# DerrickXuNu/CoBEVT

Hardware: AMD Instinct MI355X
Metric: bev_frames_per_sec (higher is better)
Workload: dtype bf16

## Files before the change

cobevt_amd/csrc/conv3x3.hip:

```cpp
#include <type_traits>

#include "common.hpp"
#include "f32_matrix.hpp"

namespace cobevt {

struct Conv3Params {
    const void* in;
    const void* wgt;
    const float* bias;
    const void* residual;
    void* out;
    int N, H, W, Cin;
    int Ho, Wo, Cout;
    int upsample;
    int act;
    int store_mode;
    int tiles_y, tiles_x, tiles_n;
    const void* in2 = nullptr;
    const float* bias2 = nullptr;
    int H2 = 0, W2 = 0, Cin2 = 0;
};

template <typename T, int NT, int NPX, int BN> struct Conv3Store {
    static constexpr int CH = Elem<T>::kChunk;
    static constexpr int CPP = BN / CH;
    static constexpr int ITEMS = NPX * CPP;
    static constexpr int NIT = (ITEMS + NT - 1) / NT;
    long off[NIT];
    uint4 rres[NIT];

    template <typename Coord>
    __device__ __forceinline__ void prepare(const Conv3Params& p, int tid, int n0, Coord coord) {
        const bool vec = (p.Cout % CH) == 0;
#pragma unroll
        for (int i = 0; i < NIT; ++i) {
            const int item = tid + i * NT;
            const int px = item / CPP, cj = item - px * CPP;
            const int col = n0 + cj * CH;
            int img = 0, oy = 0, ox = 0;
            rres[i] = make_uint4(0, 0, 0, 0);
            const bool ok = coord(px < NPX ? px : 0, img, oy, ox) & (item < ITEMS) & (col < p.Cout);
            const long o = (((long)img * p.Ho + oy) * p.Wo + ox) * p.Cout + col;
            off[i] = ok ? o : -1;
        }
        if (p.residual && vec) {
#pragma unroll
            for (int i = 0; i < NIT; ++i) rres[i] = *(const uint4*)((const T*)p.residual + (off[i] < 0 ? 0 : off[i]));
        }
    }

    __device__ __forceinline__ void finish(const Conv3Params& p, const float* stage, int srow, int tid, int n0) {
        T* out = (T*)p.out;
        const bool vec = (p.Cout % CH) == 0;
        float sv[NIT][CH];
#pragma unroll
        for (int i = 0; i < NIT; ++i) {
            const int item = tid + i * NT;
            const int px = item / CPP, cj = item - px * CPP;
            const float* src = stage + (px < NPX ? px : 0) * srow + cj * CH;
#pragma unroll
            for (int e = 0; e < CH; ++e) sv[i][e] = src[e];
        }
#pragma unroll
        for (int i = 0; i < NIT; ++i) {
            if (off[i] < 0) continue;
            const int item = tid + i * NT;
            const int px = item / CPP, cj = item - px * CPP;
            float v[8], rv[8];
#pragma unroll
            for (int e = 0; e < CH; ++e) v[e] = sv[i][e];
            if (vec) {
                if (p.residual) {
                    chunk_to_f32<T>(rres[i], rv);
#pragma unroll
                    for (int e = 0; e < CH; ++e) v[e] += rv[e];
                }
#pragma unroll
                for (int e = 0; e < CH; ++e) v[e] = p.act == 1 ? fmaxf(v[e], 0.f) : (p.act == 2 ? gelu_t<T>(v[e]) : v[e]);
                *(uint4*)(out + off[i]) = f32_to_chunk<T>(v);
            } else {
                const int col = n0 + cj * CH;
                for (int e = 0; e < CH && col + e < p.Cout; ++e) {
                    float x = v[e];
                    if (p.residual) x += load_elem<T>((const T*)p.residual, off[i] + e);
                    x = p.act == 1 ? fmaxf(x, 0.f) : (p.act == 2 ? gelu_t<T>(x) : x);
                    store_elem<T>(out, off[i] + e, x);
                }
            }
        }
    }
};

template <typename T, int NT, int NPX, int BN, typename Coord>
__device__ __forceinline__ void conv3_store_nhwc(const Conv3Params& p, const float* stage, int srow, int tid, int n0, Coord coord) {
    Conv3Store<T, NT, NPX, BN> st;
    st.prepare(p, tid, n0, coord);
    st.finish(p, stage, srow, tid, n0);
}

template <typename T, int BN, int KG> struct Conv3Cfg {
    static constexpr int TW = 16;
    static constexpr int TH = BN == 64 ? 16 : 8;
    static constexpr int PH = TH + 2, PW = TW + 2;
    static constexpr int PSTR = KG * 32 + 16;
    static constexpr int PROW = (PW * PSTR + 255) / 256 * 256;
    static constexpr int WSTR = KG * 32 + 16;
    static constexpr int PATCH_BYTES = PH * PROW;
    static constexpr int W_BYTES = BN * WSTR;
    static constexpr int SSTR = BN * 4 + 16;
    static constexpr int STAGE_BYTES = TH * TW * SSTR;
    static constexpr int MAIN_BYTES = PATCH_BYTES + 2 * W_BYTES;
    static constexpr int LDS_BYTES = MAIN_BYTES > STAGE_BYTES ? MAIN_BYTES : STAGE_BYTES;
};

constexpr int kConv3Threads = 512;

template <typename T, int BN, int KG>
__global__ __launch_bounds__(kConv3Threads) void conv3x3_kernel(Conv3Params p) {
    using C = Conv3Cfg<T, BN, KG>;
    constexpr int NT = kConv3Threads;
    constexpr int CH = Elem<T>::kChunk;
    constexpr int CC = KG * 32 / Elem<T>::kBytes;
    constexpr int TW = C::TW, TH = C::TH, PH = C::PH, PW = C::PW;
    constexpr int PSTR = C::PSTR, PROW = C::PROW, WSTR = C::WSTR;
    constexpr int PIECES = 2 * KG;
    constexpr int PATCH_ITEMS = PH * PW * PIECES;
    constexpr int P_IT = (PATCH_ITEMS + NT - 1) / NT;
    constexpr int W_ITEMS = BN * PIECES;
    constexpr int W_IT = (W_ITEMS + NT - 1) / NT;
    constexpr int WAVES_N = BN / 64;

    extern __shared__ __attribute__((aligned(16))) unsigned char smem[];
    unsigned char* patch = smem;
    unsigned char* wbuf = smem + C::PATCH_BYTES;

    int logical;
    {
        const int nblk = gridDim.x, bid = blockIdx.x, xcd = bid & 7, slot = bid >> 3;
        const int q = nblk >> 3, r = nblk & 7;
        logical = (xcd < r ? xcd * (q + 1) : r * (q + 1) + (xcd - r) * q) + slot;
    }
    const int tn = logical % p.tiles_n;
    int rest = logical / p.tiles_n;
    const int tx = rest % p.tiles_x; rest /= p.tiles_x;
    const int ty = rest % p.tiles_y;
    const int img = rest / p.tiles_y;
    const int oy0 = ty * TH, ox0 = tx * TW, n0 = tn * BN;

    const int tid = threadIdx.x, lane = tid & 63, wave = tid >> 6;
    const int h = lane >> 5, ql = lane & 31;
    const int wm = wave / WAVES_N, wn = wave % WAVES_N;
    const int nchunk = p.Cin / CC;
    const T* in = (const T*)p.in;
    const T* wg = (const T*)p.wgt;
    float ebias[2];
#pragma unroll
    for (int b = 0; b < 2; ++b) {
        const int c = n0 + wn * 64 + b * 32 + ql;
        ebias[b] = p.bias ? p.bias[p.bias && c < p.Cout ? c : 0] : 0.f;
        if (c >= p.Cout) ebias[b] = 0.f;
    }

    long pgoff[P_IT];
    int plds[P_IT];
    bool pzero[P_IT];
#pragma unroll
    for (int it = 0; it < P_IT; ++it) {
        const int item = tid + it * NT;
        pgoff[it] = 0;
        plds[it] = -1;
        pzero[it] = true;
        if (item < PATCH_ITEMS) {
            const int pix = item / PIECES, j = item - pix * PIECES;
            const int py = pix / PW, px = pix - py * PW;
            plds[it] = py * PROW + px * PSTR + j * 16;
            const int vy = oy0 - 1 + py, vx = ox0 - 1 + px;
            if (vy >= 0 && vy < p.Ho && vx >= 0 && vx < p.Wo) {
                const int sy = p.upsample ? (vy >> 1) : vy, sx = p.upsample ? (vx >> 1) : vx;
                pgoff[it] = (((long)img * p.H + sy) * p.W + sx) * p.Cin + j * CH;
                pzero[it] = false;
            }
        }
    }
    const T* wptr[W_IT];
    int wlds[W_IT];
    bool wzero[W_IT];
#pragma unroll
    for (int it = 0; it < W_IT; ++it) {
        const int item = (tid + it * NT) % W_ITEMS;
        const int row = item / PIECES, j = item - row * PIECES;
        const bool mine = tid + it * NT < W_ITEMS;
        wlds[it] = mine ? row * WSTR + j * 16 : -1;
        wzero[it] = n0 + row >= p.Cout;
        const int crow = n0 + row < p.Cout ? n0 + row : p.Cout - 1;
        wptr[it] = wg + ((size_t)crow * nchunk * 9 * CC + j * CH);
    }

    uint4 preg[P_IT];
    uint4 wregA[W_IT], wregB[W_IT];

    auto load_patch = [&](int chunk) {
#pragma unroll
        for (int it = 0; it < P_IT; ++it) preg[it] = *(const uint4*)(in + pgoff[it] + chunk * CC);
    };
    auto store_patch = [&]() {
#pragma unroll
        for (int it = 0; it < P_IT; ++it)
            if (plds[it] >= 0) *(uint4*)(patch + plds[it]) = pzero[it] ? make_uint4(0, 0, 0, 0) : stage_x_piece<T>(preg[it]);
    };
    auto load_w = [&](uint4 (&wreg)[W_IT], int step) {
#pragma unroll
        for (int it = 0; it < W_IT; ++it) wreg[it] = *(const uint4*)(wptr[it] + step * CC);
    };
    auto store_w = [&](const uint4 (&wreg)[W_IT], int buf) {
        unsigned char* wb = wbuf + buf * C::W_BYTES;
#pragma unroll
        for (int it = 0; it < W_IT; ++it)
            if (wlds[it] >= 0) *(uint4*)(wb + wlds[it]) = wzero[it] ? make_uint4(0, 0, 0, 0) : stage_w_piece<T>(wreg[it]);
    };

    f32x16 acc[2];
#pragma unroll
    for (int b = 0; b < 2; ++b)
#pragma unroll
        for (int r = 0; r < 16; ++r) acc[b][r] = 0.f;

    const int abase = (2 * wm + (ql >> 4)) * PROW + (ql & 15) * PSTR + h * 16;
    const int bbase = (wn * 64 + ql) * WSTR + h * 16;
    const int nsteps = nchunk * 9;

    auto body = [&](int step, int chunk, int tap, uint4 (&RI)[W_IT], uint4 (&RS)[W_IT], int buf) {
        const bool next_chunk = chunk + 1 < nchunk;
        load_w(RI, step + 2 < nsteps ? step + 2 : nsteps - 1);
        if (tap == 6 && next_chunk) load_patch(chunk + 1);
        const int kh = tap / 3, kw = tap - kh * 3;
        const unsigned char* pa = patch + kh * PROW + kw * PSTR + abase;
        const unsigned char* pb = wbuf + buf * C::W_BYTES + bbase;
#pragma unroll
        for (int g = 0; g < KG; ++g) {
            const uint4 af = *(const uint4*)(pa + g * 32);
            uint4 bf[2];
#pragma unroll
            for (int b = 0; b < 2; ++b) bf[b] = *(const uint4*)(pb + b * 32 * WSTR + g * 32);
#pragma unroll
            for (int b = 0; b < 2; ++b) mfma_kgroup_ss<T>(af, bf[b], acc[b]);
        }
        if (step + 1 < nsteps) store_w(RS, buf ^ 1);
        if (tap == 8 && next_chunk) {
            __syncthreads();
            store_patch();
        }
        __syncthreads();
    };

    load_patch(0);
    load_w(wregA, 0);
    store_patch();
    store_w(wregA, 0);
    load_w(wregB, nsteps > 1 ? 1 : 0);
    __syncthreads();
    {
        int chunk = 0, tap = 0;
        for (int step = 0; step < nsteps; step += 2) {
            body(step, chunk, tap, wregA, wregB, 0);
            if (++tap == 9) { tap = 0; ++chunk; }
            if (step + 1 < nsteps) {
                body(step + 1, chunk, tap, wregB, wregA, 1);
                if (++tap == 9) { tap = 0; ++chunk; }
            }
        }
    }

    float* stage = (float*)smem;
    constexpr int SROW = C::SSTR / 4;
#pragma unroll
    for (int b = 0; b < 2; ++b) {
        const int cl = wn * 64 + b * 32 + ql;
        const float bias = ebias[b];
#pragma unroll
        for (int r = 0; r < 16; ++r) {
            const int row = acc_row(r, lane);
            const int px = (2 * wm + (row >> 4)) * TW + (row & 15);
            stage[px * SROW + cl] = acc[b][r] + bias;
        }
    }
    __syncthreads();
    T* out = (T*)p.out;
    if (p.store_mode == 0) {
        conv3_store_nhwc<T, kConv3Threads, TH * TW, BN>(p, stage, SROW, tid, n0, [&](int px, int& im, int& oy, int& ox) {
            im = img; oy = oy0 + px / TW; ox = ox0 + (px % TW);
            return oy < p.Ho && ox < p.Wo;
        });
    } else {
        constexpr int QP = (TH / 2) * (TW / 2);
        const int ocn = BN * 4;
        const int cpp = ocn / CH;
        for (int item = tid; item < QP * cpp; item += kConv3Threads) {
            const int qp = item / cpp, cj = item - qp * cpp;
            const int qy = qp / (TW / 2), qx = qp % (TW / 2);
            const int oy2 = (oy0 >> 1) + qy, ox2 = (ox0 >> 1) + qx;
            if (oy2 >= (p.Ho >> 1) || ox2 >= (p.Wo >> 1)) continue;
            float v[8];
            bool any = false;
#pragma unroll
            for (int e = 0; e < CH; ++e) {
                const int oc = cj * CH + e, c = oc >> 2, q = oc & 3;
                const int px = (2 * qy + (q >> 1)) * TW + 2 * qx + (q & 1);
                float x = stage[px * SROW + c];
                x = p.act == 1 ? fmaxf(x, 0.f) : (p.act == 2 ? gelu_t<T>(x) : x);
                v[e] = x;
                any |= (n0 + c) < p.Cout;
            }
            if (!any) continue;
            const size_t o = (((size_t)img * (p.Ho >> 1) + oy2) * (p.Wo >> 1) + ox2) * (size_t)(p.Cout * 4) + (size_t)n0 * 4 + cj * CH;
            if (n0 + ((cj * CH + CH - 1) >> 2) < p.Cout && ((p.Cout * 4) % CH) == 0) *(uint4*)(out + o) = f32_to_chunk<T>(v);
            else for (int e = 0; e < CH; ++e) if (n0 + ((cj * CH + e) >> 2) < p.Cout) store_elem<T>(out, o + e, v[e]);
        }
    }
}

template <typename T, int BN, int KG>
static int launch_conv3(Conv3Params p, hipStream_t stream) {
    using C = Conv3Cfg<T, BN, KG>;
    p.tiles_y = (p.Ho + C::TH - 1) / C::TH;
    p.tiles_x = (p.Wo + 15) / 16;
    p.tiles_n = (p.Cout + BN - 1) / BN;
    const long blocks = (long)p.N * p.tiles_y * p.tiles_x * p.tiles_n;
    if (blocks <= 0 || blocks > 0x7fffffffL) return COBEVT_ERR_SHAPE;
    constexpr size_t lds = C::LDS_BYTES;
    cobevt::allow_dynamic_lds<conv3x3_kernel<T, BN, KG>>((int)lds);
    hipLaunchKernelGGL((conv3x3_kernel<T, BN, KG>), dim3((unsigned)blocks), dim3(kConv3Threads), lds, stream, p);
    return cobevt::launch_status();
}


#ifndef COBEVT_CONV3_PLOAD_TAP
#define COBEVT_CONV3_PLOAD_TAP 3
#endif
#ifndef COBEVT_CONV3_PSTORE_SPREAD
#define COBEVT_CONV3_PSTORE_SPREAD 1
#endif
#ifndef COBEVT_CONV3_PSTORE_FIRST
#define COBEVT_CONV3_PSTORE_FIRST 6
#endif
#ifndef COBEVT_CONV3_CONT
#define COBEVT_CONV3_CONT 1
#endif
#ifndef COBEVT_CONV3_CONT_LEAD
#define COBEVT_CONV3_CONT_LEAD 3
#endif
#ifndef COBEVT_CONV3_KNOCK
#define COBEVT_CONV3_KNOCK 0
#endif
#ifdef COBEVT_CONV3_TRACE
__device__ unsigned long long cobevt_conv3_trace[64];
__device__ unsigned long long cobevt_conv3_rt[3 * 2048];
#define COBEVT_TRACE_MARK(i) do { if (logical == 0 && tid == 0) cobevt_conv3_trace[(i)] = __builtin_readcyclecounter(); } while (0)
#define COBEVT_TRACE_RT(i) do { if (threadIdx.x == 0 && blockIdx.x < 2048) cobevt_conv3_rt[blockIdx.x * 3 + (i)] = (i) == 2 ? (unsigned long long)(__builtin_amdgcn_s_getreg((20 << 0) | (0 << 6) | (3 << 11)) & 15) : __builtin_amdgcn_s_memrealtime(); } while (0)
#else
#define COBEVT_TRACE_MARK(i) do {} while (0)
#define COBEVT_TRACE_RT(i) do {} while (0)
#endif

template <typename T, int MT, int WN, int KS, int S = 1, int NW = 8> struct Conv3SCfg {
    static constexpr int NT = 64 * NW, KG = 4, KGW = KG / KS;
    static constexpr bool HALF = NW == 4;
    static constexpr int BN = WN * 32;
    static constexpr int PW = S == 1 ? 18 : 33;
    static constexpr int SROWS = S == 1 ? 4 : 5;
    static constexpr int PSTR = KG * 32 + 16;
    static constexpr int PLANE = 17 * PSTR;
    static constexpr int PROW = ((S == 1 ? PW * PSTR : 2 * PLANE) + 255) / 256 * 256;
    static constexpr int STRIP_BYTES = SROWS * PROW;
    static constexpr int PATCH_BYTES = MT * STRIP_BYTES;
    static constexpr int SSTR = BN * 4 + 16;
    static constexpr int STAGE_BYTES = MT * 32 * SSTR;
    static constexpr int MAIN_BYTES = (S == 1 && !HALF ? 2 : 1) * PATCH_BYTES;
    static constexpr int LDS_BYTES = MAIN_BYTES > STAGE_BYTES ? MAIN_BYTES : STAGE_BYTES;
    static_assert(WN * KS == NW && (NW == 8 || (NW == 4 && S == 1)), "eight waves, or four (stride 1)");
};

template <typename T, int MT, int WN, int KS, int S, int NW, bool DS = false>
__global__ __launch_bounds__(64 * NW, NW == 4 ? 2 : 1) void conv3x3_strips_kernel(Conv3Params p) {
    static_assert(!DS || (Elem<T>::kIsBf16 && S == 1 && NW == 8), "the shortcut form is bf16 / stride 1 / eight waves");
    using C = Conv3SCfg<T, MT, WN, KS, S, NW>;
    constexpr bool HALF = C::HALF;
    constexpr int NT = C::NT, KG = C::KG, KGW = C::KGW, BN = C::BN, PW = C::PW;
    constexpr int CH = Elem<T>::kChunk;
    constexpr int CC = KG * 32 / Elem<T>::kBytes;
    constexpr int PSTR = C::PSTR, PROW = C::PROW, STRIP = C::STRIP_BYTES;
    constexpr int PIECES = 2 * KG;
    constexpr int STRIP_ITEMS = C::SROWS * PW * PIECES;
    constexpr int PATCH_ITEMS = MT * STRIP_ITEMS;
    constexpr int P_IT = S == 1 ? (PATCH_ITEMS + NT - 1) / NT : 1;
    constexpr int PF = 2, R = 3;
    constexpr bool PACK = kXPack<T, KGW>;
    constexpr bool PACK3 = kXPack3<T, KGW>;
    constexpr int KGA = (PACK || PACK3) ? KGW / 2 : KGW;
    constexpr int RA = PACK3 ? 2 : 3;
    constexpr bool CONT = COBEVT_CONV3_CONT && S == 1 && !HALF && Elem<T>::kIsBf16 && (KGA == 1 || KGA == 2) && MT <= 5;
    constexpr int TB = CONT ? (9 * KGA - 2) / KGA : 9;

    extern __shared__ __attribute__((aligned(16))) unsigned char smem[];
    unsigned char* patch = smem;
    COBEVT_TRACE_RT(0);
    COBEVT_TRACE_RT(2);

    int logical;
    {
        const int nblk = gridDim.x, bid = blockIdx.x, xcd = bid & 7, slot = bid >> 3;
        const int q = nblk >> 3, r = nblk & 7;
        logical = (xcd < r ? xcd * (q + 1) : r * (q + 1) + (xcd - r) * q) + slot;
    }
    const int tn = logical % p.tiles_n;
    const int q0 = (logical / p.tiles_n) * MT;
    const int n0 = tn * BN;
    const int per_img = p.tiles_y * p.tiles_x;
    const int nstrips = p.N * per_img;

    const int tid = threadIdx.x, lane = tid & 63, wave = tid >> 6;
    const int h = lane >> 5, ql = lane & 31;
    const int wn = wave % WN, ks = wave / WN;
    const int nchunk = p.Cin / CC;
    const int nchunk2 = DS ? p.Cin2 / CC : 0;
    const int nsteps = nchunk * 9 + nchunk2;
    const T* in = (const T*)p.in;

    __shared__ __attribute__((aligned(16))) int stab[8 * 4];
    __shared__ __attribute__((aligned(16))) float sbias[BN];
    __shared__ __attribute__((aligned(16))) float sbias2[DS ? BN : 4];
    if (tid >= NT - BN) {
        const int c = n0 + tid - (NT - BN);
        sbias[tid - (NT - BN)] = (p.bias && c < p.Cout) ? p.bias[c] : 0.f;
        if (DS) sbias2[tid - (NT - BN)] = (p.bias2 && c < p.Cout) ? p.bias2[c] : 0.f;
    }
    if (tid < MT) {
        const int q = q0 + tid;
        const bool ok = q < nstrips;
        const int img = ok ? q / per_img : 0, rem = ok ? q - img * per_img : 0;
        const int sy = rem / p.tiles_x, sx = rem - sy * p.tiles_x;
        *(int4*)&stab[tid * 4] = make_int4(img, sy, sx, ok ? 1 : 0);
    }
    __syncthreads();

    int pgoff[P_IT];
    int plds[P_IT];
#pragma unroll
    for (int it = 0; it < P_IT; ++it) {
        const int item = tid + it * NT;
        pgoff[it] = 0;
        plds[it] = -1;
        if (S == 1 && item < PATCH_ITEMS) {
            const int s = item / STRIP_ITEMS, r = item - s * STRIP_ITEMS;
            const int pix = r / PIECES, j = r - pix * PIECES;
            const int py = pix / PW, px = pix - py * PW;
            int lds = s * STRIP + py * PROW + px * PSTR + (PACK ? packed_piece_offset(j) : PACK3 ? packed3_piece_offset(j) : j * 16);
            const int4 sc = *(const int4*)&stab[s * 4];
            const int img = sc.x, sy = sc.y, sx = sc.z;
            const int vy = sy * 2 - 1 + py, vx = sx * 16 - 1 + px;
            const bool valid = (sc.w != 0) & (vy >= 0) & (vy < p.Ho) & (vx >= 0) & (vx < p.Wo);
            const int yy = p.upsample ? (vy >> 1) : vy, xx = p.upsample ? (vx >> 1) : vx;
            pgoff[it] = valid ? ((img * p.H + yy) * p.W + xx) * p.Cin + j * CH : 0;
            plds[it] = valid ? lds : (lds | (1 << 30));
        }
    }
    const uint4* wq = (const uint4*)p.wgt + ((size_t)(n0 / 32 + wn) * nsteps) * (KG * 64) + ks * KGW * 64 + lane;

    uint4 preg[P_IT];
    auto load_patch = [&](int chunk) {
#pragma unroll
        for (int it = 0; it < P_IT; ++it) preg[it] = *(const uint4*)(in + pgoff[it] + chunk * CC);
    };
    auto store_patch = [&](unsigned char* dst) {
#pragma unroll
        for (int it = 0; it < P_IT; ++it)
            if (plds[it] >= 0) {
                if constexpr (PACK) *(uint2*)(dst + (plds[it] & 0x3fffffff)) = (plds[it] >> 30) ? make_uint2(0, 0) : pack_f16_hi(preg[it]);
                else if constexpr (PACK3) store_piece_packed3(dst + (plds[it] & 0x3fffffff), preg[it], (plds[it] >> 30) != 0);
                else *(uint4*)(dst + (plds[it] & 0x3fffffff)) = (plds[it] >> 30) ? make_uint4(0, 0, 0, 0) : stage_x_piece<T>(preg[it]);
            }
    };
    constexpr int PSF = CONT ? TB - 3 : COBEVT_CONV3_PSTORE_FIRST;
    constexpr int PSN = TB - PSF;
    auto store_patch_part = [&](unsigned char* dst, int part) {
#pragma unroll
        for (int it = 0; it < P_IT; ++it)
            if (it % PSN == part && plds[it] >= 0) {
                if constexpr (PACK) *(uint2*)(dst + (plds[it] & 0x3fffffff)) = (plds[it] >> 30) ? make_uint2(0, 0) : pack_f16_hi(preg[it]);
                else if constexpr (PACK3) store_piece_packed3(dst + (plds[it] & 0x3fffffff), preg[it], (plds[it] >> 30) != 0);
                else *(uint4*)(dst + (plds[it] & 0x3fffffff)) = (plds[it] >> 30) ? make_uint4(0, 0, 0, 0) : stage_x_piece<T>(preg[it]);
            }
    };
    auto load_b = [&](uint4 (&b)[KGW], int step) {
#pragma unroll
        for (int g = 0; g < KGW; ++g) b[g] = wq[(size_t)step * (KG * 64) + g * 64];
    };
    auto fill_patch_s2 = [&](int chunk) {
        constexpr int BATCH = 8;
        for (int base = 0; base < PATCH_ITEMS; base += BATCH * NT) {
            uint4 v[BATCH];
            int dst[BATCH];
#pragma unroll
            for (int u = 0; u < BATCH; ++u) {
                const int item = base + u * NT + tid;
                dst[u] = -1;
                v[u] = make_uint4(0, 0, 0, 0);
                if (item < PATCH_ITEMS) {
                    const int st = item / STRIP_ITEMS, r = item - st * STRIP_ITEMS;
                    const int pix = r / PIECES, j = r - pix * PIECES;
                    const int py = pix / PW, px = pix - py * PW;
                    dst[u] = st * STRIP + py * PROW + (px & 1) * C::PLANE + (px >> 1) * PSTR + (PACK ? packed_piece_offset(j) : PACK3 ? packed3_piece_offset(j) : j * 16);
                    const int4 sc = *(const int4*)&stab[st * 4];
                    if (sc.w) {
                        const int img = sc.x, sy = sc.y, sx = sc.z;
                        const int vy = sy * 4 - 1 + py, vx = sx * 32 - 1 + px;
                        if (vy >= 0 && vy < p.H && vx >= 0 && vx < p.W)
                            v[u] = *(const uint4*)(in + ((img * p.H + vy) * p.W + vx) * p.Cin + j * CH + chunk * CC);
                    }
                }
            }
#pragma unroll
            for (int u = 0; u < BATCH; ++u)
                if (dst[u] >= 0) {
                    if constexpr (PACK) *(uint2*)(patch + dst[u]) = pack_f16_hi(v[u]);
                    else if constexpr (PACK3) store_piece_packed3(patch + dst[u], v[u], false);
                    else *(uint4*)(patch + dst[u]) = stage_x_piece<T>(v[u]);
                }
        }
    };

    f32x16 acc[MT];
#pragma unroll
    for (int a = 0; a < MT; ++a)
#pragma unroll
        for (int r = 0; r < 16; ++r) acc[a][r] = 0.f;

    const int abase = (ql >> 4) * S * PROW + (ql & 15) * PSTR + (PACK3 ? h * 32 + ks * KGA * 64 : h * 16 + ks * KGA * 32);

    uint4 bq[R][KGW];
    COBEVT_TRACE_MARK(0);
    if (S == 1) load_patch(0);
#pragma unroll
    for (int s = 0; s < PF; ++s) load_b(bq[s], s < nsteps ? s : nsteps - 1);
    float* stage = (float*)smem;
    constexpr int SROW = C::SSTR / 4;
    auto reduce_ksplit = [&](const float* bias_lds, bool trace) {
        const int c0 = wn * 32 + 4 * h;
        float4 bias4[4];
#pragma unroll
        for (int k = 0; k < 4; ++k) bias4[k] = *(const float4*)&bias_lds[c0 + 8 * k];
        if (trace) COBEVT_TRACE_MARK(57);
#pragma unroll
        for (int r = 0; r < KS; ++r) {
#pragma unroll
            for (int a = 0; a < MT; ++a) {
                if (((a + KS - r) % KS) != ks) continue;
#pragma unroll
                for (int k = 0; k < 4; ++k) {
                    float4* d = (float4*)(stage + (a * 32 + ql) * SROW + c0 + 8 * k);
                    float4 v = make_float4(acc[a][4 * k], acc[a][4 * k + 1], acc[a][4 * k + 2], acc[a][4 * k + 3]);
                    if (r == 0) {
                        v.x += bias4[k].x; v.y += bias4[k].y; v.z += bias4[k].z; v.w += bias4[k].w;
                    } else {
                        const float4 o = *d;
                        v.x += o.x; v.y += o.y; v.z += o.z; v.w += o.w;
                    }
                    *d = v;
                }
            }
            __syncthreads();
            if (trace && r == 0) COBEVT_TRACE_MARK(58);
        }
    };
    if (S == 1) store_patch(patch);
    else fill_patch_s2(0);
    __syncthreads();
    COBEVT_TRACE_MARK(1);
    constexpr bool EARLY_RES = S == 1 && Elem<T>::kIsBf16 && MT <= 5;
    Conv3Store<T, NT, MT * 32, BN> st;
    auto coord = [&](int px, int& im, int& oy, int& ox) {
        const int4 sc = *(const int4*)&stab[(px >> 5) * 4];
        im = sc.x;
        oy = sc.y * 2 + ((px >> 4) & 1); ox = sc.z * 16 + (px & 15);
        return (sc.w != 0) & (oy < p.Ho) & (ox < p.Wo);
    };
    constexpr int PLT = (S == 1 && !HALF) ? (CONT ? PSF - COBEVT_CONV3_CONT_LEAD : COBEVT_CONV3_PLOAD_TAP) : 0;
    uint4 af[RA][MT];
    uint4 al[PACK3 ? RA : 1][PACK3 ? MT : 1];
    auto read_a_from = [&](const unsigned char* pb, int slot, int n) {
        const int t2 = n / KGA, g2 = n - t2 * KGA;
        const int kh2 = t2 / 3, kw2 = t2 - kh2 * 3;
        const int toff = S == 1 ? kh2 * PROW + kw2 * PSTR : kh2 * PROW + (kw2 & 1) * C::PLANE + (kw2 >> 1) * PSTR;
        const unsigned char* pn = pb + toff + abase + g2 * (PACK3 ? 64 : 32);
#pragma unroll
        for (int a = 0; a < MT; ++a) {
            af[slot][a] = *(const uint4*)(pn + a * STRIP);
            if constexpr (PACK3) al[slot][a] = *(const uint4*)(pn + a * STRIP + 16);
        }
    };
    if (CONT) {
        read_a_from(patch, 0, 0);
        read_a_from(patch, 1, 1);
        __builtin_amdgcn_sched_barrier(0);
    }
    auto run_chunk = [&](int chunk, auto last_tag) {
        constexpr bool LAST = decltype(last_tag)::value;
        const bool more = chunk + 1 < nchunk;
        unsigned char* pbuf = patch + (S == 1 && !HALF ? (chunk & 1) * C::PATCH_BYTES : 0);
        unsigned char* pother = patch + (S == 1 && !HALF ? ((chunk & 1) ^ 1) * C::PATCH_BYTES : 0);
        if (S == 1 && PLT == 0 && !(COBEVT_CONV3_KNOCK & 8)) load_patch(more ? chunk + 1 : chunk);
        constexpr int NG = 9 * KGA;
        auto read_a = [&](int slot, int n) { read_a_from(pbuf, slot, n); };
        if (!CONT) {
            read_a(0, 0);
            if (RA == 3) read_a(1, 1);
            __builtin_amdgcn_sched_barrier(0);
        }
#pragma unroll
        for (int tap = 0; tap < 9; ++tap) {
            const int step = chunk * 9 + tap;
            if (chunk < 4) COBEVT_TRACE_MARK(2 + chunk * 9 + tap);
            if (CONT && tap == TB) {
                __syncthreads();
                __builtin_amdgcn_sched_barrier(0);
            }
#ifdef COBEVT_CONV3_SETPRIO
            if ((tap ^ ks) & 1) __builtin_amdgcn_s_setprio(3); else __builtin_amdgcn_s_setprio(0);
#endif
            if (!(COBEVT_CONV3_KNOCK & 1) || chunk == 0)
                load_b(bq[(tap + PF) % R], step + PF < nsteps ? step + PF : nsteps - 1);
            if (S == 1 && PLT > 0 && tap == PLT) {
                if (LAST) { if (EARLY_RES && p.store_mode == 0) st.prepare(p, tid, n0, coord); }
                else if (!(COBEVT_CONV3_KNOCK & 8)) load_patch(more ? chunk + 1 : chunk);
            }
            __builtin_amdgcn_sched_barrier(0);
#pragma unroll
            for (int g = 0; g < KGA; ++g) {
                const int n = tap * KGA + g;
                if (n + RA - 1 < NG) { if (!(COBEVT_CONV3_KNOCK & 4) || chunk == 0) read_a((n + RA - 1) % RA, n + RA - 1); }
                else if (CONT && !LAST && !(COBEVT_CONV3_KNOCK & 4)) read_a_from(pother, (n + RA - 1) % RA, n + RA - 1 - NG);
                uint4 wpk = make_uint4(0, 0, 0, 0), wlo = make_uint4(0, 0, 0, 0);
                if constexpr (PACK) wpk = pack_f16_pair(bq[tap % R][(2 * g) % KGW], bq[tap % R][(2 * g + 1) % KGW]);
                if constexpr (PACK3) split_w_pair(bq[tap % R][(2 * g) % KGW], bq[tap % R][(2 * g + 1) % KGW], wpk, wlo);
#pragma unroll
                for (int a = 0; a < MT; ++a) {
                    if (COBEVT_CONV3_KNOCK & 2) acc[a][0] += __uint_as_float((af[n % RA][a].x ^ bq[tap % R][g].x) & 0x3fffffffu);
                    else if constexpr (PACK) mfma_f16_packed(wpk, af[n % RA][a], acc[a]);
                    else if constexpr (PACK3) mfma_3term(wpk, wlo, af[n % RA][a], al[PACK3 ? n % RA : 0][PACK3 ? a : 0], acc[a]);
                    else mfma_kgroup_xs<T>(bq[tap % R][g], af[n % RA][a], acc[a]);
                }
                if (Elem<T>::kIsBf16 && (n + 2 < NG || (CONT && !LAST))) {
#pragma unroll
                    for (int a = 0; a < MT; ++a) {
                        __builtin_amdgcn_sched_group_barrier(0x100, 1, 0);
                        __builtin_amdgcn_sched_group_barrier(0x008, 1, 0);
                    }
                }
                __builtin_amdgcn_sched_barrier(0);
            }
            if (S == 1 && !HALF && more && !LAST && !(COBEVT_CONV3_KNOCK & 8)) {
                if (COBEVT_CONV3_PSTORE_SPREAD || CONT) {
                    if (tap >= PSF && tap < TB) { store_patch_part(pother, tap - PSF); __builtin_amdgcn_sched_barrier(0); }
                } else if (tap == 6) {
                    store_patch(pother);
                    __builtin_amdgcn_sched_barrier(0);
                }
            }
        }
        if (chunk < 4) COBEVT_TRACE_MARK(41 + 2 * chunk);
#ifdef COBEVT_CONV3_TRACE
        if (logical == 0 && lane == 0 && chunk == 0) {
            cobevt_conv3_trace[49 + wave] = __builtin_readcyclecounter();
            cobevt_conv3_trace[57 + wave > 63 ? 63 : 57 + wave] = 0;
            unsigned hw = __builtin_amdgcn_s_getreg((4 << 0) | (0 << 6) | (31 << 11));
            cobevt_conv3_trace[49 + wave] |= (unsigned long long)((hw >> 4) & 3) << 60;
        }
#endif
        if (!CONT) __syncthreads();
        if (HALF && more) {
            store_patch(pbuf);
            __syncthreads();
        }
        if (chunk < 4) COBEVT_TRACE_MARK(42 + 2 * chunk);
    };
    constexpr int XI = MT * 32 * PIECES, X_IT = DS ? (XI + NT - 1) / NT : 1, XCH = MT * 32 * PSTR;
    int xoff[X_IT], xlds[X_IT];
    const T* in2 = (const T*)p.in2;
    uint4 xr[2][X_IT];
    auto load_x = [&](uint4 (&x)[X_IT], int e) {
#pragma unroll
        for (int it = 0; it < X_IT; ++it) x[it] = *(const uint4*)(in2 + xoff[it] + e * CC);
    };
    auto store_x = [&](const uint4 (&x)[X_IT], int e) {
#pragma unroll
        for (int it = 0; it < X_IT; ++it)
            if (xlds[it] >= 0) *(uint4*)(patch + e * XCH + (xlds[it] & 0x3fffffff)) = (xlds[it] >> 30) ? make_uint4(0, 0, 0, 0) : x[it];
    };
    if (S == 1) {
        for (int chunk = 0; chunk + 1 < nchunk; ++chunk) run_chunk(chunk, std::false_type{});
        if constexpr (DS) {
#pragma unroll
            for (int it = 0; it < X_IT; ++it) {
                const int item = tid + it * NT;
                xoff[it] = 0;
                xlds[it] = -1;
                if (item < XI) {
                    const int pi = item / PIECES, j = item - pi * PIECES;
                    const int4 sc = *(const int4*)&stab[(pi >> 5) * 4];
                    const int oy = sc.y * 2 + ((pi >> 4) & 1), ox = sc.z * 16 + (pi & 15);
                    const bool valid = (sc.w != 0) & (oy < p.Ho) & (ox < p.Wo);
                    xoff[it] = valid ? ((sc.x * p.H2 + 2 * oy) * p.W2 + 2 * ox) * p.Cin2 + j * CH : 0;
                    xlds[it] = (pi * PSTR + j * 16) | (valid ? 0 : (1 << 30));
                }
            }
            load_x(xr[0], 0);
            load_x(xr[1], nchunk2 > 1 ? 1 : 0);
        }
        if (PLT == 0 && EARLY_RES && p.store_mode == 0) st.prepare(p, tid, n0, coord);
        __builtin_amdgcn_sched_barrier(0);
        run_chunk(nchunk - 1, std::true_type{});
    } else {
#pragma unroll 1
        for (int chunk = 0; chunk < nchunk; ++chunk) {
            if (chunk > 0) {
                fill_patch_s2(chunk);
                __syncthreads();
            }
            run_chunk(chunk, std::false_type{});
        }
    }
    if constexpr (DS) {
        for (int e0 = 0; e0 < nchunk2; e0 += 2) {
            if (e0 > 0) {
                load_x(xr[0], e0);
                load_x(xr[1], e0 + 1 < nchunk2 ? e0 + 1 : e0);
            }
            store_x(xr[0], e0);
            if (e0 + 1 < nchunk2) store_x(xr[1], e0 + 1);
        }
        __syncthreads();
        {
            const int c0 = wn * 32 + 4 * h;
            float4 bias4[4];
#pragma unroll
            for (int k = 0; k < 4; ++k) bias4[k] = *(const float4*)&sbias2[c0 + 8 * k];
            const uint4* wd = (const uint4*)p.wgt + ((size_t)(n0 / 32 + wn) * nsteps + nchunk * 9) * (KG * 64) + lane;
            uint4 bw[4][KG];
#pragma unroll
            for (int e = 0; e < 4; ++e)
                if (e < nchunk2) {
#pragma unroll
                    for (int g = 0; g < KG; ++g) bw[e][g] = wd[(size_t)e * (KG * 64) + g * 64];
                }
#pragma unroll
            for (int a = 0; a < MT; ++a) {
                if ((a % KS) != ks) continue;
                f32x16 dacc;
#pragma unroll
                for (int r = 0; r < 16; ++r) dacc[r] = 0.f;
                const unsigned char* xa = patch + (a * 32 + ql) * PSTR + h * 16;
#pragma unroll
                for (int e = 0; e < 4; ++e) {
                    if (e >= nchunk2) continue;
                    uint4 ax[KG];
#pragma unroll
                    for (int g = 0; g < KG; ++g) ax[g] = *(const uint4*)(xa + e * XCH + g * 32);
#pragma unroll
                    for (int g = 0; g < KG; ++g) mfma_kgroup_xs<T>(bw[e][g], ax[g], dacc);
                }
#pragma unroll
                for (int k = 0; k < 4; ++k) {
                    const uint32_t lo = pack_bf2(dacc[4 * k] + bias4[k].x, dacc[4 * k + 1] + bias4[k].y);
                    const uint32_t hi = pack_bf2(dacc[4 * k + 2] + bias4[k].z, dacc[4 * k + 3] + bias4[k].w);
                    acc[a][4 * k] += __uint_as_float(lo << 16);
                    acc[a][4 * k + 1] += __uint_as_float(lo & 0xffff0000u);
                    acc[a][4 * k + 2] += __uint_as_float(hi << 16);
                    acc[a][4 * k + 3] += __uint_as_float(hi & 0xffff0000u);
                }
            }
        }
        __syncthreads();
    }
    COBEVT_TRACE_MARK(38);

    reduce_ksplit(sbias, true);
    COBEVT_TRACE_MARK(39);
    T* out = (T*)p.out;
    if (p.store_mode == 0) {
        if (!EARLY_RES) st.prepare(p, tid, n0, coord);
        st.finish(p, stage, SROW, tid, n0);
    } else {
        const int cpp = BN * 4 / CH;
        for (int item = tid; item < MT * 8 * cpp; item += NT) {
            const int qp = item / cpp, cj = item - qp * cpp;
            const int s = qp >> 3, qx = qp & 7;
            const int4 sc = *(const int4*)&stab[s * 4];
            if (!sc.w) continue;
            const int img = sc.x, sy = sc.y, sx = sc.z;
            const int oy2 = sy, ox2 = sx * 8 + qx;
            if (oy2 >= (p.Ho >> 1) || ox2 >= (p.Wo >> 1)) continue;
            float v[8];
            bool any = false;
#pragma unroll
            for (int e = 0; e < CH; ++e) {
                const int oc = cj * CH + e, c = oc >> 2, qd = oc & 3;
                const int px = s * 32 + (qd >> 1) * 16 + 2 * qx + (qd & 1);
                float x = stage[px * SROW + c];
                x = p.act == 1 ? fmaxf(x, 0.f) : (p.act == 2 ? gelu_t<T>(x) : x);
                v[e] = x;
                any |= (n0 + c) < p.Cout;
            }
            if (!any) continue;
            const size_t o = (((size_t)img * (p.Ho >> 1) + oy2) * (p.Wo >> 1) + ox2) * (size_t)(p.Cout * 4) + (size_t)n0 * 4 + cj * CH;
            if (n0 + ((cj * CH + CH - 1) >> 2) < p.Cout && ((p.Cout * 4) % CH) == 0) *(uint4*)(out + o) = f32_to_chunk<T>(v);
            else for (int e = 0; e < CH; ++e) if (n0 + ((cj * CH + e) >> 2) < p.Cout) store_elem<T>(out, o + e, v[e]);
        }
    }
    COBEVT_TRACE_MARK(40);
    COBEVT_TRACE_RT(1);
}

template <typename T, int MT, int WN, int KS, int S, int NW = 8, bool DS = false>
static int launch_conv3s(Conv3Params p, int coutp, hipStream_t stream) {
    using C = Conv3SCfg<T, MT, WN, KS, S, NW>;
    if ((long)p.N * p.H * p.W * p.Cin >= 0x7fffffffL) return COBEVT_ERR_UNSUPPORTED;
    if (DS && (long)p.N * p.H2 * p.W2 * p.Cin2 >= 0x7fffffffL) return COBEVT_ERR_UNSUPPORTED;
    if (DS && (long)(p.Cin2 / 64) * MT * 32 * C::PSTR > (long)C::LDS_BYTES) return COBEVT_ERR_UNSUPPORTED;
    p.tiles_y = (p.Ho + 1) / 2;
    p.tiles_x = (p.Wo + 15) / 16;
    p.tiles_n = (p.Cout + C::BN - 1) / C::BN;
    if (p.tiles_n * C::BN > coutp) return COBEVT_ERR_SHAPE;
    const long nstrips = (long)p.N * p.tiles_y * p.tiles_x;
    const long blocks = (nstrips + MT - 1) / MT * p.tiles_n;
    if (blocks <= 0 || blocks > 0x7fffffffL) return COBEVT_ERR_SHAPE;
    constexpr size_t lds = C::LDS_BYTES;
    cobevt::allow_dynamic_lds<conv3x3_strips_kernel<T, MT, WN, KS, S, NW, DS>>((int)lds);
    hipLaunchKernelGGL((conv3x3_strips_kernel<T, MT, WN, KS, S, NW, DS>), dim3((unsigned)blocks), dim3(C::NT), lds, stream, p);
    return cobevt::launch_status();
}

template <typename T, int MT>
static int launch_conv3s_bn(const Conv3Params& p, int coutp, int bn64, int stride, hipStream_t stream) {
    if constexpr (Elem<T>::kIsBf16 && MT <= 5) {
        if (bn64 == 3 && stride == 1) return launch_conv3s<T, MT, 1, 4, 1, 4>(p, coutp, stream);
    }
    if (bn64 > 1) return COBEVT_ERR_UNSUPPORTED;
    if (stride == 2) return bn64 ? launch_conv3s<T, MT, 2, 4, 2>(p, coutp, stream) : launch_conv3s<T, MT, 4, 2, 2>(p, coutp, stream);
    return bn64 ? launch_conv3s<T, MT, 2, 4, 1>(p, coutp, stream) : launch_conv3s<T, MT, 4, 2, 1>(p, coutp, stream);
}

template <typename T>
static int dispatch_conv3f(const Conv3Params& p, int kg, int coutp, int variant, int stride, hipStream_t stream) {
    if (kg != 4) return COBEVT_ERR_UNSUPPORTED;
    if (variant == 0) variant = p.Cout <= 64 ? 151 : 150;
    const int mt = (variant - 100) / 10, bn64 = (variant - 100) % 10;
    if (variant < 100 || bn64 > 3) return COBEVT_ERR_ARG;
    if constexpr (Elem<T>::kIsBf16) {
        if (bn64 == 3 && stride == 1 && mt == 1) return launch_conv3s<T, 1, 1, 4, 1, 4>(p, coutp, stream);
        if (bn64 == 3 && stride == 1 && mt == 2) return launch_conv3s<T, 2, 1, 4, 1, 4>(p, coutp, stream);
    }
    switch (mt) {
        case 3: return launch_conv3s_bn<T, 3>(p, coutp, bn64, stride, stream);
        case 4: return launch_conv3s_bn<T, 4>(p, coutp, bn64, stride, stream);
        case 5: return launch_conv3s_bn<T, 5>(p, coutp, bn64, stride, stream);
        case 6: return launch_conv3s_bn<T, 6>(p, coutp, bn64, stride, stream);
        default: return COBEVT_ERR_ARG;
    }
}

}

using namespace cobevt;

extern "C" int cobevt_conv3x3_nhwc(const void* in, const void* wgt, const float* bias, const void* residual, void* out,
                                   const int* dims, hipStream_t stream) {
    if (!in || !wgt || !out || !dims) return COBEVT_ERR_ARG;
    Conv3Params p;
    const int dtype = dims[0];
    p.in = in; p.wgt = wgt; p.bias = bias; p.residual = residual; p.out = out;
    p.N = dims[1]; p.H = dims[2]; p.W = dims[3]; p.Cin = dims[4]; p.Cout = dims[5];
    p.upsample = dims[6]; p.act = dims[7]; p.store_mode = dims[8];
    const int cc = dims[9];
    p.Ho = p.upsample ? 2 * p.H : p.H;
    p.Wo = p.upsample ? 2 * p.W : p.W;
    if (dtype != 0 && dtype != 1) return COBEVT_ERR_ARG;
    if (p.N < 1 || p.H < 1 || p.W < 1 || p.Cin < 1 || p.Cout < 1) return COBEVT_ERR_SHAPE;
    if (p.store_mode != 0 && p.store_mode != 1) return COBEVT_ERR_ARG;
    if (p.store_mode == 1 && (p.residual || ((p.Ho | p.Wo) & 1))) return COBEVT_ERR_UNSUPPORTED;
    if (p.Cin % cc != 0) return COBEVT_ERR_SHAPE;
    const int kg = cc * (dtype == 0 ? 2 : 4) / 32;
    const bool wide = p.Cout > 64;
    if (dtype == 0) {
        if (kg == 4) return wide ? launch_conv3<bf16_t, 128, 4>(p, stream) : launch_conv3<bf16_t, 64, 4>(p, stream);
        if (kg == 2) return wide ? launch_conv3<bf16_t, 128, 2>(p, stream) : launch_conv3<bf16_t, 64, 2>(p, stream);
    } else {
        if (kg == 4) return wide ? launch_conv3<float, 128, 4>(p, stream) : launch_conv3<float, 64, 4>(p, stream);
        if (kg == 2) return wide ? launch_conv3<float, 128, 2>(p, stream) : launch_conv3<float, 64, 2>(p, stream);
    }
    return COBEVT_ERR_SHAPE;
}

extern "C" int cobevt_conv3x3_wfrag_nhwc(const void* in, const void* wfrag, const float* bias, const void* residual, void* out,
                                         const int* dims, hipStream_t stream) {
    if (!in || !wfrag || !out || !dims) return COBEVT_ERR_ARG;
    Conv3Params p;
    const int dtype = dims[0];
    p.in = in; p.wgt = wfrag; p.bias = bias; p.residual = residual; p.out = out;
    p.N = dims[1]; p.H = dims[2]; p.W = dims[3]; p.Cin = dims[4]; p.Cout = dims[5];
    p.upsample = dims[6]; p.act = dims[7]; p.store_mode = dims[8];
    const int cc = dims[9], coutp = dims[10], variant = dims[11], stride = dims[12];
    if (stride != 1 && stride != 2) return COBEVT_ERR_ARG;
    if (stride == 2 && (p.upsample || p.store_mode != 0)) return COBEVT_ERR_UNSUPPORTED;
    p.Ho = stride == 2 ? (p.H - 1) / 2 + 1 : (p.upsample ? 2 * p.H : p.H);
    p.Wo = stride == 2 ? (p.W - 1) / 2 + 1 : (p.upsample ? 2 * p.W : p.W);
    if (dtype != 0 && dtype != 1) return COBEVT_ERR_ARG;
    if (p.N < 1 || p.H < 1 || p.W < 1 || p.Cin < 1 || p.Cout < 1 || cc < 1) return COBEVT_ERR_SHAPE;
    if (p.store_mode != 0 && p.store_mode != 1) return COBEVT_ERR_ARG;
    if (p.store_mode == 1 && (p.residual || ((p.Ho | p.Wo) & 1))) return COBEVT_ERR_UNSUPPORTED;
    if (p.Cin % cc != 0 || coutp % 32 != 0 || coutp < p.Cout) return COBEVT_ERR_SHAPE;
    const int kg = cc * (dtype == 0 ? 2 : 4) / 32;
    return dtype == 0 ? dispatch_conv3f<bf16_t>(p, kg, coutp, variant, stride, stream)
                      : dispatch_conv3f<float>(p, kg, coutp, variant, stride, stream);
}

extern "C" int cobevt_conv3x3_ds_wfrag_nhwc(const void* in, const void* in2, const void* wfrag, const float* bias, const float* bias2, void* out,
                                            const int* dims, hipStream_t stream) {
    if (!in || !in2 || !wfrag || !out || !dims) return COBEVT_ERR_ARG;
    if (dims[0] != 0) return COBEVT_ERR_UNSUPPORTED;
    Conv3Params p;
    p.in = in; p.wgt = wfrag; p.bias = bias; p.bias2 = bias2; p.residual = nullptr; p.out = out; p.in2 = in2;
    p.N = dims[1]; p.H = dims[2]; p.W = dims[3]; p.Cin = dims[4]; p.Cout = dims[5];
    p.upsample = 0; p.act = dims[6]; p.store_mode = 0;
    const int coutp = dims[7], variant = dims[8];
    p.H2 = dims[9]; p.W2 = dims[10]; p.Cin2 = dims[11];
    p.Ho = p.H; p.Wo = p.W;
    if (p.N < 1 || p.H < 1 || p.W < 1 || p.Cin < 64 || p.Cin % 64 || p.Cout < 1 || p.Cin2 < 64 || p.Cin2 % 64) return COBEVT_ERR_SHAPE;
    if (p.Cin2 > 256) return COBEVT_ERR_UNSUPPORTED;
    if ((p.H2 - 1) / 2 + 1 != p.H || (p.W2 - 1) / 2 + 1 != p.W) return COBEVT_ERR_SHAPE;
    if (coutp % 32 != 0 || coutp < p.Cout) return COBEVT_ERR_SHAPE;
    if (p.act < 0 || p.act > 2) return COBEVT_ERR_ARG;
    const int mt = (variant - 100) / 10, bn64 = (variant - 100) % 10;
    if (variant < 100 || bn64 > 1) return COBEVT_ERR_ARG;
    switch (mt * 2 + bn64) {
        case 6: return launch_conv3s<bf16_t, 3, 4, 2, 1, 8, true>(p, coutp, stream);
        case 7: return launch_conv3s<bf16_t, 3, 2, 4, 1, 8, true>(p, coutp, stream);
        case 8: return launch_conv3s<bf16_t, 4, 4, 2, 1, 8, true>(p, coutp, stream);
        case 9: return launch_conv3s<bf16_t, 4, 2, 4, 1, 8, true>(p, coutp, stream);
        case 10: return launch_conv3s<bf16_t, 5, 4, 2, 1, 8, true>(p, coutp, stream);
        case 11: return launch_conv3s<bf16_t, 5, 2, 4, 1, 8, true>(p, coutp, stream);
        default: return COBEVT_ERR_UNSUPPORTED;
    }
}

#ifdef COBEVT_CONV3_TRACE
extern "C" int cobevt_conv3_read_trace(unsigned long long* dst) {
    return hipMemcpyFromSymbol(dst, HIP_SYMBOL(cobevt_conv3_trace), sizeof(unsigned long long) * 64) == hipSuccess ? 0 : 1;
}
extern "C" int cobevt_conv3_read_rt(unsigned long long* dst) {
    return hipMemcpyFromSymbol(dst, HIP_SYMBOL(cobevt_conv3_rt), sizeof(unsigned long long) * 3 * 2048) == hipSuccess ? 0 : 1;
}
#endif
```

Measured before the change: 598.9.

## Double-buffer stride-2 conv3x3 patches and add wide-tile geometry selector

Adds a DB2 mode for bf16 stride-2 3x3 convolutions. It prefetches the input patch into registers and stores it into a second LDS buffer while the current chunk computes, the same way the stride-1 path already works. A new selector also remaps some stride-2 variants (MT 5/6 with Cout a multiple of 256) to a 3-strip, 8-wave-wide N tile with one K split. This is meant to hide global-load latency and the patch-fill stall in the downsampling convs, at the cost of double LDS usage and more registers for the prefetch.

After: 593.3. Within noise of the previous version (-0.9%).

```diff
diff --git a/cobevt_amd/csrc/conv3_select.hpp b/cobevt_amd/csrc/conv3_select.hpp
--- /dev/null
+++ b/cobevt_amd/csrc/conv3_select.hpp
@@ -0,0 +1,30 @@
+#pragma once
+#include "../../include/cobevt_hip.h"
+
+namespace cobevt {
+
+struct Conv3Request {
+    bool bf16;
+    int stride;
+    int nchunk;
+    int cout, coutp;
+    long nstrips;
+    int variant;
+};
+
+struct Conv3Geom { int status, MT, WN, KS, NW; bool DB2; };
+
+inline Conv3Geom conv3_select(const Conv3Request& r) {
+    const auto fail = [](int code) { return Conv3Geom{code, 0, 0, 0, 0, false}; };
+    const int variant = r.variant == 0 ? (r.cout <= 64 ? 151 : 150) : r.variant;
+    const int mt = (variant - 100) / 10, code = (variant - 100) % 10;
+    if (variant < 100 || code > 3) return fail(COBEVT_ERR_ARG);
+    if (r.bf16 && code == 3 && r.stride == 1 && mt >= 1 && mt <= 5) return Conv3Geom{COBEVT_OK, mt, 1, 4, 4, false};
+    if (mt < 3 || mt > 6) return fail(COBEVT_ERR_ARG);
+    if (code > 1) return fail(COBEVT_ERR_UNSUPPORTED);
+    if (r.bf16 && r.stride == 2 && r.coutp % 256 == 0 && r.nchunk >= 2 && (mt == 5 || mt == 6)) return Conv3Geom{COBEVT_OK, 3, 8, 1, 8, true};
+    const bool db2 = r.bf16 && r.stride == 2 && mt == 3 && r.nchunk >= 2;
+    return code ? Conv3Geom{COBEVT_OK, mt, 2, 4, 8, db2} : Conv3Geom{COBEVT_OK, mt, 4, 2, 8, db2};
+}
+
+}
diff --git a/cobevt_amd/csrc/conv3x3.hip b/cobevt_amd/csrc/conv3x3.hip
--- a/cobevt_amd/csrc/conv3x3.hip
+++ b/cobevt_amd/csrc/conv3x3.hip
@@ -1,6 +1,7 @@
 #include <type_traits>
 
 #include "common.hpp"
+#include "conv3_select.hpp"
 #include "f32_matrix.hpp"
 
 namespace cobevt {
@@ -363,7 +364,7 @@
 #define COBEVT_TRACE_RT(i) do {} while (0)
 #endif
 
-template <typename T, int MT, int WN, int KS, int S = 1, int NW = 8> struct Conv3SCfg {
+template <typename T, int MT, int WN, int KS, int S = 1, int NW = 8, bool DB2 = false> struct Conv3SCfg {
     static constexpr int NT = 64 * NW, KG = 4, KGW = KG / KS;
     static constexpr bool HALF = NW == 4;
     static constexpr int BN = WN * 32;
@@ -376,15 +377,18 @@
     static constexpr int PATCH_BYTES = MT * STRIP_BYTES;
     static constexpr int SSTR = BN * 4 + 16;
     static constexpr int STAGE_BYTES = MT * 32 * SSTR;
-    static constexpr int MAIN_BYTES = (S == 1 && !HALF ? 2 : 1) * PATCH_BYTES;
+    static constexpr bool S2DB = DB2;
+    static_assert(!DB2 || (S == 2 && MT <= 3 && Elem<T>::kIsBf16), "two stride-2 patch buffers: bf16, at most three strips");
+    static constexpr bool DBUF = (S == 1 && !HALF) || S2DB;
+    static constexpr int MAIN_BYTES = (DBUF ? 2 : 1) * PATCH_BYTES;
     static constexpr int LDS_BYTES = MAIN_BYTES > STAGE_BYTES ? MAIN_BYTES : STAGE_BYTES;
     static_assert(WN * KS == NW && (NW == 8 || (NW == 4 && S == 1)), "eight waves, or four (stride 1)");
 };
 
-template <typename T, int MT, int WN, int KS, int S, int NW, bool DS = false>
+template <typename T, int MT, int WN, int KS, int S, int NW, bool DS = false, bool DB2 = false>
 __global__ __launch_bounds__(64 * NW, NW == 4 ? 2 : 1) void conv3x3_strips_kernel(Conv3Params p) {
     static_assert(!DS || (Elem<T>::kIsBf16 && S == 1 && NW == 8), "the shortcut form is bf16 / stride 1 / eight waves");
-    using C = Conv3SCfg<T, MT, WN, KS, S, NW>;
+    using C = Conv3SCfg<T, MT, WN, KS, S, NW, DB2>;
     constexpr bool HALF = C::HALF;
     constexpr int NT = C::NT, KG = C::KG, KGW = C::KGW, BN = C::BN, PW = C::PW;
     constexpr int CH = Elem<T>::kChunk;
@@ -393,7 +397,9 @@
     constexpr int PIECES = 2 * KG;
     constexpr int STRIP_ITEMS = C::SROWS * PW * PIECES;
     constexpr int PATCH_ITEMS = MT * STRIP_ITEMS;
-    constexpr int P_IT = S == 1 ? (PATCH_ITEMS + NT - 1) / NT : 1;
+    constexpr bool DBUF = C::DBUF;
+    constexpr bool PRE = S == 1 || C::S2DB;
+    constexpr int P_IT = PRE ? (PATCH_ITEMS + NT - 1) / NT : 1;
     constexpr int PF = 2, R = 3;
     constexpr bool PACK = kXPack<T, KGW>;
     constexpr bool PACK3 = kXPack3<T, KGW>;
@@ -451,15 +457,16 @@
         const int item = tid + it * NT;
         pgoff[it] = 0;
         plds[it] = -1;
-        if (S == 1 && item < PATCH_ITEMS) {
+        if (PRE && item < PATCH_ITEMS) {
             const int s = item / STRIP_ITEMS, r = item - s * STRIP_ITEMS;
             const int pix = r / PIECES, j = r - pix * PIECES;
             const int py = pix / PW, px = pix - py * PW;
-            int lds = s * STRIP + py * PROW + px * PSTR + (PACK ? packed_piece_offset(j) : PACK3 ? packed3_piece_offset(j) : j * 16);
+            int lds = s * STRIP + py * PROW + (S == 1 ? px * PSTR : (px & 1) * C::PLANE + (px >> 1) * PSTR)
+                    + (PACK ? packed_piece_offset(j) : PACK3 ? packed3_piece_offset(j) : j * 16);
             const int4 sc = *(const int4*)&stab[s * 4];
             const int img = sc.x, sy = sc.y, sx = sc.z;
-            const int vy = sy * 2 - 1 + py, vx = sx * 16 - 1 + px;
-            const bool valid = (sc.w != 0) & (vy >= 0) & (vy < p.Ho) & (vx >= 0) & (vx < p.Wo);
+            const int vy = sy * 2 * S - 1 + py, vx = sx * 16 * S - 1 + px;
+            const bool valid = (sc.w != 0) & (vy >= 0) & (vy < (S == 1 ? p.Ho : p.H)) & (vx >= 0) & (vx < (S == 1 ? p.Wo : p.W));
             const int yy = p.upsample ? (vy >> 1) : vy, xx = p.upsample ? (vx >> 1) : vx;
             pgoff[it] = valid ? ((img * p.H + yy) * p.W + xx) * p.Cin + j * CH : 0;
             plds[it] = valid ? lds : (lds | (1 << 30));
@@ -540,7 +547,7 @@
 
     uint4 bq[R][KGW];
     COBEVT_TRACE_MARK(0);
-    if (S == 1) load_patch(0);
+    if (PRE) load_patch(0);
 #pragma unroll
     for (int s = 0; s < PF; ++s) load_b(bq[s], s < nsteps ? s : nsteps - 1);
     float* stage = (float*)smem;
@@ -573,7 +580,7 @@
             if (trace && r == 0) COBEVT_TRACE_MARK(58);
         }
     };
-    if (S == 1) store_patch(patch);
+    if (PRE) store_patch(patch);
     else fill_patch_s2(0);
     __syncthreads();
     COBEVT_TRACE_MARK(1);
@@ -585,7 +592,7 @@
         oy = sc.y * 2 + ((px >> 4) & 1); ox = sc.z * 16 + (px & 15);
         return (sc.w != 0) & (oy < p.Ho) & (ox < p.Wo);
     };
-    constexpr int PLT = (S == 1 && !HALF) ? (CONT ? PSF - COBEVT_CONV3_CONT_LEAD : COBEVT_CONV3_PLOAD_TAP) : 0;
+    constexpr int PLT = DBUF ? (CONT ? PSF - COBEVT_CONV3_CONT_LEAD : COBEVT_CONV3_PLOAD_TAP) : 0;
     uint4 af[RA][MT];
     uint4 al[PACK3 ? RA : 1][PACK3 ? MT : 1];
     auto read_a_from = [&](const unsigned char* pb, int slot, int n) {
@@ -607,9 +614,9 @@
     auto run_chunk = [&](int chunk, auto last_tag) {
         constexpr bool LAST = decltype(last_tag)::value;
         const bool more = chunk + 1 < nchunk;
-        unsigned char* pbuf = patch + (S == 1 && !HALF ? (chunk & 1) * C::PATCH_BYTES : 0);
-        unsigned char* pother = patch + (S == 1 && !HALF ? ((chunk & 1) ^ 1) * C::PATCH_BYTES : 0);
-        if (S == 1 && PLT == 0 && !(COBEVT_CONV3_KNOCK & 8)) load_patch(more ? chunk + 1 : chunk);
+        unsigned char* pbuf = patch + (DBUF ? (chunk & 1) * C::PATCH_BYTES : 0);
+        unsigned char* pother = patch + (DBUF ? ((chunk & 1) ^ 1) * C::PATCH_BYTES : 0);
+        if (PRE && PLT == 0 && !(COBEVT_CONV3_KNOCK & 8)) load_patch(more ? chunk + 1 : chunk);
         constexpr int NG = 9 * KGA;
         auto read_a = [&](int slot, int n) { read_a_from(pbuf, slot, n); };
         if (!CONT) {
@@ -630,7 +637,7 @@
 #endif
             if (!(COBEVT_CONV3_KNOCK & 1) || chunk == 0)
                 load_b(bq[(tap + PF) % R], step + PF < nsteps ? step + PF : nsteps - 1);
-            if (S == 1 && PLT > 0 && tap == PLT) {
+            if (PRE && PLT > 0 && tap == PLT) {
                 if (LAST) { if (EARLY_RES && p.store_mode == 0) st.prepare(p, tid, n0, coord); }
                 else if (!(COBEVT_CONV3_KNOCK & 8)) load_patch(more ? chunk + 1 : chunk);
             }
@@ -659,7 +666,7 @@
                 }
                 __builtin_amdgcn_sched_barrier(0);
             }
-            if (S == 1 && !HALF && more && !LAST && !(COBEVT_CONV3_KNOCK & 8)) {
+            if (DBUF && more && !LAST && !(COBEVT_CONV3_KNOCK & 8)) {
                 if (COBEVT_CONV3_PSTORE_SPREAD || CONT) {
                     if (tap >= PSF && tap < TB) { store_patch_part(pother, tap - PSF); __builtin_amdgcn_sched_barrier(0); }
                 } else if (tap == 6) {
@@ -697,7 +704,7 @@
         for (int it = 0; it < X_IT; ++it)
             if (xlds[it] >= 0) *(uint4*)(patch + e * XCH + (xlds[it] & 0x3fffffff)) = (xlds[it] >> 30) ? make_uint4(0, 0, 0, 0) : x[it];
     };
-    if (S == 1) {
+    if (PRE) {
         for (int chunk = 0; chunk + 1 < nchunk; ++chunk) run_chunk(chunk, std::false_type{});
         if constexpr (DS) {
 #pragma unroll
@@ -821,9 +828,9 @@
     COBEVT_TRACE_RT(1);
 }
 
-template <typename T, int MT, int WN, int KS, int S, int NW = 8, bool DS = false>
+template <typename T, int MT, int WN, int KS, int S, int NW = 8, bool DS = false, bool DB2 = false>
 static int launch_conv3s(Conv3Params p, int coutp, hipStream_t stream) {
-    using C = Conv3SCfg<T, MT, WN, KS, S, NW>;
+    using C = Conv3SCfg<T, MT, WN, KS, S, NW, DB2>;
     if ((long)p.N * p.H * p.W * p.Cin >= 0x7fffffffL) return COBEVT_ERR_UNSUPPORTED;
     if (DS && (long)p.N * p.H2 * p.W2 * p.Cin2 >= 0x7fffffffL) return COBEVT_ERR_UNSUPPORTED;
     if (DS && (long)(p.Cin2 / 64) * MT * 32 * C::PSTR > (long)C::LDS_BYTES) return COBEVT_ERR_UNSUPPORTED;
@@ -835,36 +842,42 @@
     const long blocks = (nstrips + MT - 1) / MT * p.tiles_n;
     if (blocks <= 0 || blocks > 0x7fffffffL) return COBEVT_ERR_SHAPE;
     constexpr size_t lds = C::LDS_BYTES;
-    cobevt::allow_dynamic_lds<conv3x3_strips_kernel<T, MT, WN, KS, S, NW, DS>>((int)lds);
-    hipLaunchKernelGGL((conv3x3_strips_kernel<T, MT, WN, KS, S, NW, DS>), dim3((unsigned)blocks), dim3(C::NT), lds, stream, p);
+    cobevt::allow_dynamic_lds<conv3x3_strips_kernel<T, MT, WN, KS, S, NW, DS, DB2>>((int)lds);
+    hipLaunchKernelGGL((conv3x3_strips_kernel<T, MT, WN, KS, S, NW, DS, DB2>), dim3((unsigned)blocks), dim3(C::NT), lds, stream, p);
     return cobevt::launch_status();
 }
 
 template <typename T, int MT>
-static int launch_conv3s_bn(const Conv3Params& p, int coutp, int bn64, int stride, hipStream_t stream) {
+static int launch_conv3s_geom(const Conv3Params& p, int coutp, const Conv3Geom& g, int stride, hipStream_t stream) {
     if constexpr (Elem<T>::kIsBf16 && MT <= 5) {
-        if (bn64 == 3 && stride == 1) return launch_conv3s<T, MT, 1, 4, 1, 4>(p, coutp, stream);
-    }
-    if (bn64 > 1) return COBEVT_ERR_UNSUPPORTED;
-    if (stride == 2) return bn64 ? launch_conv3s<T, MT, 2, 4, 2>(p, coutp, stream) : launch_conv3s<T, MT, 4, 2, 2>(p, coutp, stream);
-    return bn64 ? launch_conv3s<T, MT, 2, 4, 1>(p, coutp, stream) : launch_conv3s<T, MT, 4, 2, 1>(p, coutp, stream);
+        if (g.NW == 4) return launch_conv3s<T, MT, 1, 4, 1, 4>(p, coutp, stream);
+    }
+    if constexpr (Elem<T>::kIsBf16 && MT == 3) {
+        if (g.DB2 && g.WN == 8) return launch_conv3s<T, 3, 8, 1, 2, 8, false, true>(p, coutp, stream);
+        if (g.DB2 && g.WN == 4) return launch_conv3s<T, 3, 4, 2, 2, 8, false, true>(p, coutp, stream);
+        if (g.DB2 && g.WN == 2) return launch_conv3s<T, 3, 2, 4, 2, 8, false, true>(p, coutp, stream);
+    }
+    if (g.DB2 || g.WN == 8) return COBEVT_ERR_UNSUPPORTED;
+    if constexpr (MT >= 3) {
+        if (g.NW == 8 && g.WN == 2) return stride == 2 ? launch_conv3s<T, MT, 2, 4, 2>(p, coutp, stream) : launch_conv3s<T, MT, 2, 4, 1>(p, coutp, stream);
+        if (g.NW == 8 && g.WN == 4) return stride == 2 ? launch_conv3s<T, MT, 4, 2, 2>(p, coutp, stream) : launch_conv3s<T, MT, 4, 2, 1>(p, coutp, stream);
+    }
+    return COBEVT_ERR_UNSUPPORTED;
 }
 
 template <typename T>
 static int dispatch_conv3f(const Conv3Params& p, int kg, int coutp, int variant, int stride, hipStream_t stream) {
     if (kg != 4) return COBEVT_ERR_UNSUPPORTED;
-    if (variant == 0) variant = p.Cout <= 64 ? 151 : 150;
-    const int mt = (variant - 100) / 10, bn64 = (variant - 100) % 10;
-    if (variant < 100 || bn64 > 3) return COBEVT_ERR_ARG;
-    if constexpr (Elem<T>::kIsBf16) {
-        if (bn64 == 3 && stride == 1 && mt == 1) return launch_conv3s<T, 1, 1, 4, 1, 4>(p, coutp, stream);
-        if (bn64 == 3 && stride == 1 && mt == 2) return launch_conv3s<T, 2, 1, 4, 1, 4>(p, coutp, stream);
-    }
-    switch (mt) {
-        case 3: return launch_conv3s_bn<T, 3>(p, coutp, bn64, stride, stream);
-        case 4: return launch_conv3s_bn<T, 4>(p, coutp, bn64, stride, stream);
-        case 5: return launch_conv3s_bn<T, 5>(p, coutp, bn64, stride, stream);
-        case 6: return launch_conv3s_bn<T, 6>(p, coutp, bn64, stride, stream);
+    const long nstrips = (long)p.N * ((p.Ho + 1) / 2) * ((p.Wo + 15) / 16);
+    const Conv3Geom g = conv3_select(Conv3Request{Elem<T>::kIsBf16, stride, p.Cin / (128 / Elem<T>::kBytes), p.Cout, coutp, nstrips, variant});
+    if (g.status != COBEVT_OK) return g.status;
+    switch (g.MT) {
+        case 1: return launch_conv3s_geom<T, 1>(p, coutp, g, stride, stream);
+        case 2: return launch_conv3s_geom<T, 2>(p, coutp, g, stride, stream);
+        case 3: return launch_conv3s_geom<T, 3>(p, coutp, g, stride, stream);
+        case 4: return launch_conv3s_geom<T, 4>(p, coutp, g, stride, stream);
+        case 5: return launch_conv3s_geom<T, 5>(p, coutp, g, stride, stream);
+        case 6: return launch_conv3s_geom<T, 6>(p, coutp, g, stride, stream);
         default: return COBEVT_ERR_ARG;
     }
 }
```
